# martius-lab/iCEM

Hardware: AMD Instinct MI355X
Metric: traj-steps/sec (N x h), iCEM inner planning loop (higher is better)
Workload: dtype f32 storage; model step 2xfp16 planes (3 products), f32 accumulate

## Files before the change

### icem_amd/csrc/k_merge.hip

```cpp
#include "fused_dev.h"
#include "refit.h"
#include "update_small_body.h"

namespace icem {

namespace {

template <int KREG, bool REC, int KX = 0>
__device__ __forceinline__ void merge_single_body(const MergeSingleArgs& a, unsigned char* smem_raw) {
    __shared__ unsigned long long sel[64];
    __shared__ unsigned long long cand[64];
    __shared__ int slot[64];
    typedef float __attribute__((address_space(3))) * LdsF;
    const LdsF new_mean = (LdsF)smem_raw;
    const int tid = threadIdx.x;
    const int lane = tid & 63;
    const int hd = a.h * a.d;
    if (a.dbg && threadIdx.x == 0) a.dbg[0] = wall_clock64();
    constexpr int EPL = 4;
    const bool pre = hd <= MERGE_WG * EPL;
    float om[EPL], os[EPL], blo[EPL], bhi[EPL];
#pragma unroll
    for (int i = 0; i < EPL; ++i) {
        const int e = tid + i * MERGE_WG;
        om[i] = (pre && e < hd) ? a.mean[e] : 0.f;
        os[i] = (pre && e < hd) ? a.std[e] : 0.f;
    }
    auto request_bounds = [&]() {
#pragma unroll
        for (int i = 0; i < EPL; ++i) {
            const int e = tid + i * MERGE_WG;
            blo[i] = (pre && a.last && e < hd) ? a.low[e % a.d] : 0.f;
            bhi[i] = (pre && a.last && e < hd) ? a.high[e % a.d] : 0.f;
        }
    };
    if (REC || tid >= 64) request_bounds();
    if constexpr (REC) {
        merge_select_records_wg(a, tid < 64, lane, tid, MERGE_WG, sel, slot);
        if (a.dbg && threadIdx.x == 0) a.dbg[4] = wall_clock64();
    } else {
        if (tid < 64) merge_select_shallow<3>(a, lane, cand, sel);
        if (a.dbg && threadIdx.x == 0) a.dbg[4] = wall_clock64();
        if (tid < 64) request_bounds();
        __syncthreads();
    }
    const float* rows[KREG];
    constexpr int NR = KX > 0 ? KX : KREG;
    merge_rows<KREG, REC, KX>(a, sel, slot, rows);
    float best0 = 0.f;
    auto finish_one = [&](int e, float old_mean, float old_std) {
        float xs[KREG];
#pragma unroll
        for (int r = 0; r < NR; ++r) xs[r] = rows[r][e];
#pragma unroll
        for (int r = 0; r < NR; ++r) asm volatile("" : "+v"(xs[r]));
        float nm, ns;
        refit_element_regs<float, KREG, KX>(a.K, a.alpha, old_mean, old_std, xs, nm, ns);
#pragma unroll
        for (int r = 0; r < NR; ++r)
            if (KX > 0 || r < a.K) a.elites_next[(size_t)r * hd + e] = xs[r];
        if (!a.last) {
            a.mean_out[e] = nm;
            a.std_out[e] = ns;
        } else {
            new_mean[e] = nm;
        }
        if (e == tid) best0 = xs[0];
    };
    if (pre) {
#pragma unroll
        for (int i = 0; i < EPL; ++i) {
            const int e = tid + i * MERGE_WG;
            if (e < hd) finish_one(e, om[i], os[i]);
        }
    } else {
        for (int e = tid; e < hd; e += MERGE_WG) finish_one(e, a.mean[e], a.std[e]);
    }
    if (a.dbg && threadIdx.x == 0) a.dbg[5] = wall_clock64();
    if (tid < (KX > 0 ? KX : a.K)) a.elites_cost_next[tid] = key_cost(sel[tid]);
    if (a.last) {
        __syncthreads();
        if (pre) {
#pragma unroll
            for (int i = 0; i < EPL; ++i) {
                const int e = tid + i * MERGE_WG;
                if (e < hd) {
                    a.mean_out[e] = (e + a.d < hd) ? new_mean[e + a.d] : new_mean[e];
                    a.std_out[e] = (bhi[i] - blo[i]) / 2.f * a.init_std;
                }
            }
        } else {
            for (int e = tid; e < hd; e += MERGE_WG) {
                const int j = e % a.d;
                a.mean_out[e] = (e + a.d < hd) ? new_mean[e + a.d] : new_mean[e];
                a.std_out[e] = (a.high[j] - a.low[j]) / 2.f * a.init_std;
            }
        }
        if (tid < a.d) a.executed[tid] = best0;
        if (tid == 0) a.best_cost[0] = key_cost(sel[0]);
    }
    if (a.dbg && threadIdx.x == 0) a.dbg[6] = wall_clock64();
}

template <int KREG, bool REC>
__global__ __launch_bounds__(MERGE_WG) void merge_single_kernel(MergeSingleArgs a) {
    extern __shared__ __attribute__((aligned(16))) unsigned char smem_raw[];
    merge_single_body<KREG, REC>(a, smem_raw);
}

template <int KREG, int KX>
__global__ __launch_bounds__(MERGE_WG) void merge_single_exactk_kernel(MergeSingleArgs a) {
    extern __shared__ __attribute__((aligned(16))) unsigned char smem_raw[];
    merge_single_body<KREG, false, KX>(a, smem_raw);
}

template <int H, int KREG, int KX>
__device__ __forceinline__ void merge_noise_body(const MergeSingleArgs& a, const FastSampleArgs& z1, const FastSampleArgs& z2, int wgs1,
                                                 unsigned char* smem_raw) {
    if (blockIdx.x == 0) {
        merge_single_body<KREG, false, KX>(a, smem_raw);
        return;
    }
    const bool second = (int)blockIdx.x > wgs1;
    const FastSampleArgs& z = second ? z2 : z1;
    float* tile = reinterpret_cast<float*>(smem_raw);
    const int d = z.d, hd = H * d, tpw = MERGE_WG / d, tid = threadIdx.x;
    const int n_base = ((int)blockIdx.x - 1 - (second ? wgs1 : 0)) * tpw;
    const int n_here = cmin(tpw, z.n - n_base);
    if (tid < n_here * d) {
        const int nl = tid / d;
        const int j = tid - nl * d;
        float* trow = tile + nl * hd + j;
        sample_row<H, 10>(z.W, (unsigned)(z.first_index + n_base + nl), (unsigned)j, z.off_lo, z.off_hi, z.seed_lo, z.seed_hi,
                          [&](int t, float y) { trow[t * d] = y; }, z.white != 0);
    }
    __syncthreads();
    float* gdst = z.out + (size_t)n_base * hd;
    const int total = n_here * hd;
    if ((hd & 3) == 0) {
        const float4* t4 = reinterpret_cast<const float4*>(tile);
        float4* g4 = reinterpret_cast<float4*>(gdst);
        for (int e = tid; e < total / 4; e += MERGE_WG) g4[e] = t4[e];
    } else {
        for (int e = tid; e < total; e += MERGE_WG) gdst[e] = tile[e];
    }
}
template <int H, int KREG>
__global__ __launch_bounds__(MERGE_WG) void merge_noise_kernel(MergeSingleArgs a, FastSampleArgs z1, FastSampleArgs z2, int wgs1) {
    extern __shared__ __attribute__((aligned(16))) unsigned char smem_raw[];
    merge_noise_body<H, KREG, 0>(a, z1, z2, wgs1, smem_raw);
}
template <int H, int KREG, int KX>
__global__ __launch_bounds__(MERGE_WG) void merge_noise_exactk_kernel(MergeSingleArgs a, FastSampleArgs z1, FastSampleArgs z2, int wgs1) {
    extern __shared__ __attribute__((aligned(16))) unsigned char smem_raw[];
    merge_noise_body<H, KREG, KX>(a, z1, z2, wgs1, smem_raw);
}

template <int H, int KREG>
__global__ __launch_bounds__(MERGE_WG) void merge_noise_batch_kernel(const MergeNoiseBatchArgs* __restrict__ args, BatchBases bases, int wgs1) {
    extern __shared__ __attribute__((aligned(16))) unsigned char smem_raw[];
    const MergeNoiseBatchArgs& g = args[blockIdx.y];
    if (blockIdx.x == 0) {
        const MergeSingleArgs a = from_device(g.a);
        merge_single_body<KREG, false>(a, smem_raw);
        return;
    }
    const bool second = (int)blockIdx.x > wgs1;
    const FastSampleArgs z = from_device(second ? g.z2 : g.z1);
    float* tile = reinterpret_cast<float*>(smem_raw);
    const int d = z.d, hd = H * d, tpw = MERGE_WG / d, tid = threadIdx.x;
    const int n_base = ((int)blockIdx.x - 1 - (second ? wgs1 : 0)) * tpw;
    const int n_here = cmin(tpw, z.n - n_base);
    if (n_here <= 0) return;
    uint32_t off_lo = z.off_lo, off_hi = z.off_hi;
    add_base64(off_lo, off_hi, bases.v[blockIdx.y]);
    if (tid < n_here * d) {
        const int nl = tid / d;
        const int j = tid - nl * d;
        float* trow = tile + nl * hd + j;
        sample_row<H, 10>(z.W, (unsigned)(z.first_index + n_base + nl), (unsigned)j, off_lo, off_hi, z.seed_lo, z.seed_hi,
                          [&](int t, float y) { trow[t * d] = y; }, z.white != 0);
    }
    __syncthreads();
    float* gdst = z.out + (size_t)n_base * hd;
    const int total = n_here * hd;
    if ((hd & 3) == 0) {
        const float4* t4 = reinterpret_cast<const float4*>(tile);
        float4* g4 = reinterpret_cast<float4*>(gdst);
        for (int e = tid; e < total / 4; e += MERGE_WG) g4[e] = t4[e];
    } else {
        for (int e = tid; e < total; e += MERGE_WG) gdst[e] = tile[e];
    }
}

constexpr size_t PACK_STAGE_MAX = 48 * 1024;

template <int KREG>
__global__ __launch_bounds__(MERGE_WG) void pack_records_kernel(MergeSingleArgs a, int n_loc, int shard_lo, float* records, XchgPush px) {
    __shared__ unsigned long long sel[64];
    __shared__ unsigned long long cand[64];
    extern __shared__ __attribute__((aligned(16))) float stage[];
    const int tid = threadIdx.x;
    if (tid < 64) merge_select<KREG>(a, tid, cand, sel);
    __syncthreads();
    pack_records_body<KREG>(a, n_loc, shard_lo, records, px, stage, sel, tid, MERGE_WG);
}

template <int KREG>
__global__ __launch_bounds__(MERGE_WG) void pack_merge_kernel(MergeSingleArgs pk, int n_loc, int shard_lo, float* records, XchgPush px,
                                                               MergeSingleArgs m) {
    __shared__ unsigned long long sel[64];
    __shared__ unsigned long long cand[64];
    extern __shared__ __attribute__((aligned(16))) unsigned char smem_raw[];
    const int tid = threadIdx.x;
    if (tid < 64) merge_select<KREG>(pk, tid, cand, sel);
    __syncthreads();
    pack_records_body<KREG>(pk, n_loc, shard_lo, records, px, reinterpret_cast<float*>(smem_raw), sel, tid, MERGE_WG);
    __syncthreads();
    merge_single_body<KREG, true>(m, smem_raw);
}

__global__ __launch_bounds__(1024) void topk_small_kernel(const float* costs, int n, int K, float* out_c, int* out_i) {
    __shared__ unsigned long long wg_keys[2][16][32];
    const int lane = threadIdx.x & 63, wave = threadIdx.x >> 6;
    unsigned long long run = KEY_SENTINEL;
    bool first = true;
    for (int base = wave * 64; base < n; base += 1024) {
        const int i = base + lane;
        unsigned long long key = wave_sort64(i < n ? make_key(costs[i], i) : KEY_SENTINEL, lane);
        if (!first) {
            const unsigned long long prev = __shfl(run, lane - 32, 64);
            key = (lane >= 32 && lane < 32 + K) ? prev : (lane < K ? key : KEY_SENTINEL);
            key = wave_sort64(key, lane);
        }
        run = key;
        first = false;
    }
    FastRolloutArgs fr{};
    fr.part_c = out_c;
    fr.part_i = out_i;
    wg_merge_emit<16>(wg_keys, run, K, lane, wave, fr, 0, 1);
}

__global__ __launch_bounds__(1024) void update_small_kernel(UpdateSmallArgs a) {
    update_small_body<false>(a, nullptr);
}

template <bool FINISH>
__global__ __launch_bounds__(1024) void update_small_batch_kernel(const UpdateFinishArgs* __restrict__ args) {
    const UpdateFinishArgs g = args[blockIdx.x];
    update_small_body<FINISH>(g.u, &g);
}

}

void launch_update_small(const UpdateSmallArgs& a, hipStream_t st) {
    hipLaunchKernelGGL(update_small_kernel, dim3(1), dim3(1024), 0, st, a);
}

void launch_update_small_batch(const UpdateFinishArgs* args_dev, int n, bool finish, hipStream_t st) {
    if (finish) hipLaunchKernelGGL(update_small_batch_kernel<true>, dim3(n), dim3(1024), 0, st, args_dev);
    else hipLaunchKernelGGL(update_small_batch_kernel<false>, dim3(n), dim3(1024), 0, st, args_dev);
}

bool topk_small_ok(int n, int K) { return n >= 1 && n <= 16384 && K >= 1 && K <= 32; }

void launch_topk_small(const float* costs, int n, int K, float* out_c, int* out_i, hipStream_t st) {
    hipLaunchKernelGGL(topk_small_kernel, dim3(1), dim3(1024), 0, st, costs, n, K, out_c, out_i);
}

bool pack_can_push(int K, int h, int d) { return (size_t)K * (h * d + 2) * sizeof(float) <= PACK_STAGE_MAX; }

void launch_pack_records(const MergeSingleArgs& a, int n_loc, int shard_lo, float* records, hipStream_t st, const XchgPush& px) {
    const size_t lds = px.peers ? (size_t)a.K * (a.h * a.d + 2) * sizeof(float) : 0;
    if (a.K + 1 <= 12)
        hipLaunchKernelGGL((pack_records_kernel<12>), dim3(1), dim3(MERGE_WG), lds, st, a, n_loc, shard_lo, records, px);
    else
        hipLaunchKernelGGL((pack_records_kernel<34>), dim3(1), dim3(MERGE_WG), lds, st, a, n_loc, shard_lo, records, px);
}

void launch_pack_merge(const MergeSingleArgs& pk, int n_loc, int shard_lo, float* records, const XchgPush& px, const MergeSingleArgs& m,
                       hipStream_t st) {
    const size_t lds = std::max(px.peers ? (size_t)pk.K * (pk.h * pk.d + 2) : (size_t)0, (size_t)m.h * m.d) * sizeof(float);
    if (pk.K + 1 <= 12)
        hipLaunchKernelGGL((pack_merge_kernel<12>), dim3(1), dim3(MERGE_WG), lds, st, pk, n_loc, shard_lo, records, px, m);
    else
        hipLaunchKernelGGL((pack_merge_kernel<34>), dim3(1), dim3(MERGE_WG), lds, st, pk, n_loc, shard_lo, records, px, m);
}

bool merge_noise_ok(const MergeSingleArgs& a, int rounds) {
    return a.records == nullptr && a.K + 1 <= 12 && rounds == 10 && fast_sample_supported(a.h, a.d);
}

static LaunchKey merge_key(const MergeSingleArgs& a, const FastSampleArgs* z, const FastSampleArgs* z2) {
    LaunchKey k;
    k.family = LAUNCH_MERGE_NOISE;
    k.h = a.h, k.d = a.d, k.form = z ? 1 : 0;
    k.wgs[0] = 1;
    if (z) {
        const int tpw = MERGE_WG / z->d;
        k.wgs[1] = (z->n + tpw - 1) / tpw;
        k.wgs[2] = z2->n > 0 ? (z2->n + tpw - 1) / tpw : 0;
    }
    return k;
}
template <class F>
static bool merge_noise_dispatch(const LaunchKey& k, F&& f) {
    const size_t lds = std::max((size_t)k.h * k.d, k.form ? (size_t)(MERGE_WG / k.d) * k.h * k.d : (size_t)0) * sizeof(float);
    const int grid = k.wgs[0] + k.wgs[1] + k.wgs[2];
#define X(HH) \
    if (k.h == HH) return f(std::integral_constant<int, HH>{}, grid, lds), true;
    ICEM_FAST_HORIZONS(X)
#undef X
    return false;
}

void launch_merge_noise(const LaunchCtx& cx, const MergeSingleArgs& a, const FastSampleArgs& z, const FastSampleArgs& z2) {
    const LaunchKey k = merge_key(a, &z, &z2);
    submit(cx, k, true, [&](void* dst, unsigned long long base) { batch_form(a, &z, &z2, base, dst); }, [&] {
        merge_noise_dispatch(k, [&](auto H, int grid, size_t lds) {
            if (a.K == MERGE_EXACT_K && opt_i(OPT_MERGE_EXACT_K) != 0)
                hipLaunchKernelGGL((merge_noise_exactk_kernel<decltype(H)::value, 12, MERGE_EXACT_K>), dim3(grid), dim3(MERGE_WG), lds, cx.st, a, z, z2, k.wgs[1]);
            else
                hipLaunchKernelGGL((merge_noise_kernel<decltype(H)::value, 12>), dim3(grid), dim3(MERGE_WG), lds, cx.st, a, z, z2, k.wgs[1]);
        });
    });
}

void launch_merge_batch(const LaunchKey& k, const MergeNoiseBatchArgs* args_dev, const BatchBases& bases, int n, hipStream_t st) {
    merge_noise_dispatch(k, [&](auto H, int grid, size_t lds) {
        hipLaunchKernelGGL((merge_noise_batch_kernel<decltype(H)::value, 12>), dim3(grid, n), dim3(MERGE_WG), lds, st, args_dev, bases, k.wgs[1]);
    });
}

void launch_merge_single(const LaunchCtx& cx, const MergeSingleArgs& a) {
    const LaunchKey k = merge_key(a, nullptr, nullptr);
    submit(cx, k, !a.records && a.K + 1 <= 12, [&](void* dst, unsigned long long base) { batch_form(a, nullptr, nullptr, base, dst); }, [&] {
        const size_t lds = (size_t)a.h * a.d * sizeof(float);
        if (a.records) {
            if (a.K + 1 <= 12)
                hipLaunchKernelGGL((merge_single_kernel<12, true>), dim3(1), dim3(MERGE_WG), lds, cx.st, a);
            else
                hipLaunchKernelGGL((merge_single_kernel<34, true>), dim3(1), dim3(MERGE_WG), lds, cx.st, a);
        } else if (a.K == MERGE_EXACT_K && opt_i(OPT_MERGE_EXACT_K) != 0) {
            hipLaunchKernelGGL((merge_single_exactk_kernel<12, MERGE_EXACT_K>), dim3(1), dim3(MERGE_WG), lds, cx.st, a);
        } else if (a.K + 1 <= 12) {
            hipLaunchKernelGGL((merge_single_kernel<12, false>), dim3(1), dim3(MERGE_WG), lds, cx.st, a);
        } else {
            hipLaunchKernelGGL((merge_single_kernel<34, false>), dim3(1), dim3(MERGE_WG), lds, cx.st, a);
        }
    });
}

}
```

### icem_amd/csrc/options.h

```cpp
#pragma once

namespace icem {

#define ICEM_OPTIONS(X)                                                                                                   \
    X(DISABLE_FAST, "disable_fast", 0.0)              \
    X(FUSE_MAX_RW, "fuse_max_rw", 8.0)                \
    X(MERGE_PROLOGUE, "merge_prologue", 1.0)                                      \
    X(RIDING_PACK, "riding_pack", 1.0)                             \
    X(PUBLISHED_MERGE, "published_merge", 1.0)             \
    X(PACK_MERGE, "pack_merge", 1.0)                  \
    X(NOISE_AHEAD, "noise_ahead", 1.0)                             \
    X(NOISE_AHEAD_MIN_ROWS, "noise_ahead_min_rows", 0.0)                                                                \
    X(NOISE_AHEAD_SHARDED, "noise_ahead_sharded", 1.0)                                                                     \
    X(AHEAD_STAMPS, "ahead_stamps", 0.0)                                                                                   \
    X(AHEAD_TAIL_FRAC, "ahead_tail_frac", 0.4)                                                                             \
    X(AHEAD_NEXT1_FRAC, "ahead_next1_frac", 0.3)                                                                           \
    X(AHEAD_NOISE_LDS_KB, "ahead_noise_lds_kb", -1.0)                                                                      \
    X(MERGE_EXACT_K, "merge_exact_k", 1.0)            \
    X(PREDRAW, "predraw", 1.0)                              \
    X(GK_SAMPLE, "gk_sample", 1.0)                          \
    X(GK_ROLLOUT_THREAD, "gk_rollout_thread", 0.0)                   \
    X(GK_SELECT, "gk_select", 1.0)                                    \
    X(HN_PAIR, "hn_pair", 1.0)                                                               \
    X(HN_SPLIT, "hn_split", 1.0)                                                                                           \
    X(RSSM_SPLIT, "rssm_split", 1.0)                                                                                       \
    X(RSSM_SPLIT_MAX_N, "rssm_split_max_n", 65536.0)                                                                       \
    X(RSSM_SPLIT_TT, "rssm_split_tt", 0.0)                                                                                 \
    X(BATCH_AHEAD, "batch_ahead", 1.0)                \
    X(BATCH_AHEAD_MIN_ROWS, "batch_ahead_min_rows", 49152.0)    \
    X(BATCH_MAX_RW, "batch_max_rw", 0.0)              \
    X(LEARNED_STEP, "learned_step", 1.0)              \
    X(CEM_STEP, "cem_step", 1.0)                      \
    X(RANDOM_STEP, "random_step", 1.0)                \
    X(XCHG_LOOPBACK,"xchg_loopback", 0.0)            \
    X(XCHG_MAX_POLLS, "xchg_max_polls", 0.0)
enum Opt {
#define X(id, name, def) OPT_##id,
    ICEM_OPTIONS(X)
#undef X
    OPT_COUNT
};
constexpr int MERGE_EXACT_K = 10;
double opt(Opt k);
inline int opt_i(Opt k) { return (int)opt(k); }

}
```

Baseline: 8.653 billion.

## Split merge-noise row sampling across four threads per row with LDS-staged filter

Adds a quad variant of the merged merge+noise kernel in which four threads cooperate on each noise row: each generates a quarter of the normals and then synthesizes the colored-noise output from a filter matrix staged in shared memory. The goal is more parallelism and shorter per-thread serial sampling when the row count is small, at the cost of four times as many workgroups. It is enabled by default through a new option and only used when the grid stays within a workgroup cap. LDS sizing on the host still uses the old tile formula, and the per-row layout now depends on the row_normals_quad and row_synth_quad helpers.

Result: no change. 8.726 billion (median of 6 runs) (+0.8%).

```diff
diff --git a/icem_amd/csrc/k_merge.hip b/icem_amd/csrc/k_merge.hip
--- a/icem_amd/csrc/k_merge.hip
+++ b/icem_amd/csrc/k_merge.hip
@@ -114,7 +114,7 @@
     merge_single_body<KREG, false, KX>(a, smem_raw);
 }
 
-template <int H, int KREG, int KX>
+template <int H, int KREG, int KX, bool QUAD = false>
 __device__ __forceinline__ void merge_noise_body(const MergeSingleArgs& a, const FastSampleArgs& z1, const FastSampleArgs& z2, int wgs1,
                                                  unsigned char* smem_raw) {
     if (blockIdx.x == 0) {
@@ -124,10 +124,34 @@
     const bool second = (int)blockIdx.x > wgs1;
     const FastSampleArgs& z = second ? z2 : z1;
     float* tile = reinterpret_cast<float*>(smem_raw);
-    const int d = z.d, hd = H * d, tpw = MERGE_WG / d, tid = threadIdx.x;
+    const int d = z.d, hd = H * d, tpw = MERGE_WG / (QUAD ? 4 : 1) / d, tid = threadIdx.x;
     const int n_base = ((int)blockIdx.x - 1 - (second ? wgs1 : 0)) * tpw;
     const int n_here = cmin(tpw, z.n - n_base);
-    if (tid < n_here * d) {
+    if constexpr (QUAD) {
+        constexpr int WROWS = H / 2 + 1;
+        constexpr int WPT = (WROWS * HMAX + MERGE_WG - 1) / MERGE_WG;
+        __shared__ __attribute__((aligned(16))) float Wl[WROWS * WQ_STRIDE];
+        float wreg[WPT];
+#pragma unroll
+        for (int i = 0; i < WPT; ++i) wreg[i] = z.W[(i * MERGE_WG + tid) < WROWS * HMAX ? i * MERGE_WG + tid : 0];
+        const int rowi = tid >> 2, q = tid & 3;
+        const bool live = rowi < n_here * d;
+        const int nl = rowi / d;
+        const int j = rowi - nl * d;
+        float g[HMAX];
+        if (live)
+            row_normals_quad<H, 10>((unsigned)(z.first_index + n_base + nl), (unsigned)j, z.off_lo, z.off_hi, z.seed_lo, z.seed_hi, q, g);
+#pragma unroll
+        for (int i = 0; i < WPT; ++i) {
+            const int e = i * MERGE_WG + tid;
+            if (e < WROWS * HMAX) Wl[(e / HMAX) * WQ_STRIDE + (e % HMAX)] = wreg[i];
+        }
+        __syncthreads();
+        if (live) {
+            float* trow = tile + nl * hd + j;
+            row_synth_quad<H>(Wl, g, q, [&](int t, float y) { trow[t * d] = y; }, z.white != 0);
+        }
+    } else if (tid < n_here * d) {
         const int nl = tid / d;
         const int j = tid - nl * d;
         float* trow = tile + nl * hd + j;
@@ -154,6 +178,12 @@
 __global__ __launch_bounds__(MERGE_WG) void merge_noise_exactk_kernel(MergeSingleArgs a, FastSampleArgs z1, FastSampleArgs z2, int wgs1) {
     extern __shared__ __attribute__((aligned(16))) unsigned char smem_raw[];
     merge_noise_body<H, KREG, KX>(a, z1, z2, wgs1, smem_raw);
+}
+
+template <int H, int KREG, int KX>
+__global__ __launch_bounds__(MERGE_WG) void merge_noise_quad_kernel(MergeSingleArgs a, FastSampleArgs z1, FastSampleArgs z2, int wgs1) {
+    extern __shared__ __attribute__((aligned(16))) unsigned char smem_raw[];
+    merge_noise_body<H, KREG, KX, true>(a, z1, z2, wgs1, smem_raw);
 }
 
 template <int H, int KREG>
@@ -288,6 +318,8 @@
         hipLaunchKernelGGL((pack_merge_kernel<34>), dim3(1), dim3(MERGE_WG), lds, st, pk, n_loc, shard_lo, records, px, m);
 }
 
+constexpr int MERGE_NOISE_QUAD_MAX_WGS = 512;
+
 bool merge_noise_ok(const MergeSingleArgs& a, int rounds) {
     return a.records == nullptr && a.K + 1 <= 12 && rounds == 10 && fast_sample_supported(a.h, a.d);
 }
@@ -319,7 +351,15 @@
     const LaunchKey k = merge_key(a, &z, &z2);
     submit(cx, k, true, [&](void* dst, unsigned long long base) { batch_form(a, &z, &z2, base, dst); }, [&] {
         merge_noise_dispatch(k, [&](auto H, int grid, size_t lds) {
-            if (a.K == MERGE_EXACT_K && opt_i(OPT_MERGE_EXACT_K) != 0)
+            const bool exact_k = a.K == MERGE_EXACT_K && opt_i(OPT_MERGE_EXACT_K) != 0;
+            const int tpq = std::max(1, MERGE_WG / 4 / z.d);
+            const int wgs1 = (z.n + tpq - 1) / tpq, wgs2 = z2.n > 0 ? (z2.n + tpq - 1) / tpq : 0;
+            if (opt_i(OPT_MERGE_NOISE_QUAD) != 0 && MERGE_WG / 4 >= z.d && wgs1 + wgs2 <= MERGE_NOISE_QUAD_MAX_WGS) {
+                if (exact_k)
+                    hipLaunchKernelGGL((merge_noise_quad_kernel<decltype(H)::value, 12, MERGE_EXACT_K>), dim3(1 + wgs1 + wgs2), dim3(MERGE_WG), lds, cx.st, a, z, z2, wgs1);
+                else
+                    hipLaunchKernelGGL((merge_noise_quad_kernel<decltype(H)::value, 12, 0>), dim3(1 + wgs1 + wgs2), dim3(MERGE_WG), lds, cx.st, a, z, z2, wgs1);
+            } else if (exact_k)
                 hipLaunchKernelGGL((merge_noise_exactk_kernel<decltype(H)::value, 12, MERGE_EXACT_K>), dim3(grid), dim3(MERGE_WG), lds, cx.st, a, z, z2, k.wgs[1]);
             else
                 hipLaunchKernelGGL((merge_noise_kernel<decltype(H)::value, 12>), dim3(grid), dim3(MERGE_WG), lds, cx.st, a, z, z2, k.wgs[1]);
diff --git a/icem_amd/csrc/options.h b/icem_amd/csrc/options.h
--- a/icem_amd/csrc/options.h
+++ b/icem_amd/csrc/options.h
@@ -17,6 +17,7 @@
     X(AHEAD_NEXT1_FRAC, "ahead_next1_frac", 0.3)                                                                           \
     X(AHEAD_NOISE_LDS_KB, "ahead_noise_lds_kb", -1.0)                                                                      \
     X(MERGE_EXACT_K, "merge_exact_k", 1.0)            \
+    X(MERGE_NOISE_QUAD, "merge_noise_quad", 1.0)      \
     X(PREDRAW, "predraw", 1.0)                              \
     X(GK_SAMPLE, "gk_sample", 1.0)                          \
     X(GK_ROLLOUT_THREAD, "gk_rollout_thread", 0.0)                   \
```
